# lucidrains/magvit2-pytorch

Hardware: NVIDIA H100
Metric: video-frames/sec tokenize+decode, 17x128x128 bf16 (higher is better)
Workload: dtype bf16

## Files before the change

include/magvit2_b200.h:

```cpp
#ifndef MAGVIT2_B200_H
#define MAGVIT2_B200_H

#include <stddef.h>
#include <stdint.h>

#ifdef __cplusplus
extern "C" {
#endif

#define MV2_ABI_VERSION 4

enum { MV2_F32 = 0, MV2_BF16 = 1,
       MV2_U8 = 2    };
enum { MV2_ACT_NONE = 0, MV2_ACT_ELU = 1, MV2_ACT_SILU = 2,
       MV2_ACT_LEAKY_RELU = 3,
       MV2_ACT_RELU = 4          };
enum { MV2_SHUFFLE_NONE = 0, MV2_SHUFFLE_SPACE = 1, MV2_SHUFFLE_TIME = 2 };
enum {
  MV2_OK = 0,
  MV2_E_ARG = -1,
  MV2_E_CUDA = -2,
  MV2_E_UNSUPPORTED = -3
};

// ... 106 lines not shown
  const void* w;
  const float* bias;
  const void* res;
  void* y;
  int32_t B, Ti, Hi, Wi, Ci;
  int32_t To, Ho, Wo, Co;
  int32_t kt, kh, kw;
  int32_t st, sh, sw;
  int32_t pt, ph, pw;
  int32_t act;
  int32_t shuffle;
  int32_t epi_mode;
  const float* oscale;
  int32_t out_layout;
} mv2_tc_conv_args;
int mv2_tc_conv_supported(const mv2_tc_conv_args* a);
int mv2_tc_conv_forward(const mv2_tc_conv_args* a, void* stream);
int mv2_tc_slab_supported(const mv2_tc_conv_args* a);
int mv2_tc_slab_forward(const mv2_tc_conv_args* a, void* stream);
int mv2_tc_down_space_supported(const mv2_tc_conv_args* a);
int mv2_tc_down_space_forward(const mv2_tc_conv_args* a, void* stream);
int mv2_tc_slab_plan(const mv2_tc_conv_args* a, int n_sm, int* out6);
int mv2_tc_slab_tile(const mv2_tc_conv_args* a, int n_sm, int cta, int k, int* out6);


int mv2_dense_small(const float* x, const float* w, const float* bias, float* y, int B, int K, int N, int act, void* stream);
int mv2_mod_prepare(const float* cond, const float* S, float eps, float* scale_in, float* inv_norm, int B, int Ci, int Co,
                    void* stream);
int mv2_scale_channels(const void* x, const float* scale, void* out, int dtype, int B, int64_t positions_per_clip, int C,
                       void* stream);

typedef struct mv2_tc_ru_args {
  const void* x;
  const void* w3; const float* b3;
  const void* w1; const float* b1;
  const float* se_wk; float se_bk;
  void* y;
  float* se_ws;
  int32_t B, T, H, W, C;
  int32_t kt, kh, kw;
} mv2_tc_ru_args;
int mv2_tc_ru_supported(const mv2_tc_ru_args* a);
int mv2_tc_ru_records(const mv2_tc_ru_args* a);
size_t mv2_tc_ru_workspace_bytes(const mv2_tc_ru_args* a);
int mv2_tc_ru_forward(const mv2_tc_ru_args* a, void* stream);
int mv2_se_gate_records(const void* workspace, int nrec, int F, int C, int Hd,
// ... 25 lines not shown
```

magvit2_pytorch_b200/_lib.py:

```python
from __future__ import annotations

import ctypes as C
import os

_HERE = os.path.dirname(os.path.abspath(__file__))
LIB_PATH = os.environ.get("MV2_LIB_PATH") or os.path.join(_HERE, "libmagvit2_b200.so")

MV2_F32, MV2_BF16, MV2_U8 = 0, 1, 2
ACT_NONE, ACT_ELU, ACT_SILU, ACT_LEAKY_RELU, ACT_RELU = 0, 1, 2, 3, 4
SHUFFLE_NONE, SHUFFLE_SPACE, SHUFFLE_TIME = 0, 1, 2


class Mv2Error(RuntimeError):
    pass


class ConvArgs(C.Structure):
    _fields_ = [
        ("x", C.c_void_p), ("w", C.c_void_p), ("bias", C.c_void_p), ("res", C.c_void_p), ("y", C.c_void_p),
        ("dtype", C.c_int32),
        ("B", C.c_int32), ("Ti", C.c_int32), ("Hi", C.c_int32), ("Wi", C.c_int32), ("Ci", C.c_int32),
        ("To", C.c_int32), ("Ho", C.c_int32), ("Wo", C.c_int32), ("Co", C.c_int32),
        ("kt", C.c_int32), ("kh", C.c_int32), ("kw", C.c_int32),
        ("st", C.c_int32), ("sh", C.c_int32), ("sw", C.c_int32),
# ... 68 lines not shown
    "mv2_geglu": (_I, [_VP, _VP, _I, _I64, _I, _VP]),
    "mv2_lfq_forward": (_I, [_VP, _I, _I64, _I, _I, _I, _VP, _VP, _VP, _VP, _F, _I, _VP, _VP, _VP, _VP]),
    "mv2_lfq_decode": (_I, [_VP, _I, _I64, _I, _I, _I, _VP, _VP, _VP, _I, _VP]),
    "mv2_fsq_forward": (_I, [_VP, _I, _I64, _I, _I, _I, C.POINTER(C.c_int32), _VP, _VP, _VP, _VP, _VP, _VP, _VP, _VP]),
    "mv2_fsq_decode": (_I, [_VP, _I, _I64, _I, _I, _I, C.POINTER(C.c_int32), _VP, _VP, _VP, _I, _VP]),
    "mv2_lfq_entropy_partials": (_I, [_VP, _I64, _I, _I, _F, _VP, _VP, _VP]),
    "mv2_lfq_aux_finalize": (_I, [_VP, _VP, _I, _I, _I64, _I64, _F, _F, _F, _VP, _VP]),
    "mv2_lfq_entropy_fact_workspace_bytes": (_SZ, [_I64, _I, _I]),
    "mv2_lfq_entropy_fact_partials": (_I, [_VP, _I64, _I, _I, _F, _VP, _VP, _VP, _VP]),
    "mv2_lfq_entropy_fact_backward": (_I, [_VP, _VP, _I64, _I, _I, _F, _F, _F, _VP, _VP, _VP]),
    "mv2_gateloop_scan": (_I, [_VP, _VP, _VP, _I, _I, _I, _I, _I, _VP]),
    "mv2_mse": (_I, [_VP, _I, _VP, _I, _I64, _VP, _VP, _VP]),
    "mv2_mse_workspace_bytes": (C.c_size_t, []),
    "mv2_maxpool2x2": (_I, [_VP, _VP, _I, _I, _I, _I, _I, _VP]),
    "mv2_maxpool2x2_backward": (_I, [_VP, _VP, _VP, _I, _I, _I, _I, _I, _VP]),
    "mv2_tc_conv_supported": (_I, [C.POINTER(TcConvArgs)]),
    "mv2_tc_conv_forward": (_I, [C.POINTER(TcConvArgs), _VP]),
    "mv2_tc_slab_supported": (_I, [C.POINTER(TcConvArgs)]),
    "mv2_tc_slab_forward": (_I, [C.POINTER(TcConvArgs), _VP]),
    "mv2_tc_down_space_supported": (_I, [C.POINTER(TcConvArgs)]),
    "mv2_tc_down_space_forward": (_I, [C.POINTER(TcConvArgs), _VP]),
    "mv2_tc_slab_plan": (_I, [C.POINTER(TcConvArgs), _I, C.POINTER(C.c_int32)]),
    "mv2_tc_slab_tile": (_I, [C.POINTER(TcConvArgs), _I, _I, _I, C.POINTER(C.c_int32)]),
    "mv2_dense_small": (_I, [_VP, _VP, _VP, _VP, _I, _I, _I, _I, _VP]),
    "mv2_mod_prepare": (_I, [_VP, _VP, _F, _VP, _VP, _I, _I, _I, _VP]),
    "mv2_scale_channels": (_I, [_VP, _VP, _VP, _I, _I, _I64, _I, _VP]),
    "mv2_tc_ru_supported": (_I, [C.POINTER(TcRuArgs)]),
    "mv2_tc_ru_records": (_I, [C.POINTER(TcRuArgs)]),
    "mv2_tc_ru_workspace_bytes": (_SZ, [C.POINTER(TcRuArgs)]),
    "mv2_tc_ru_forward": (_I, [C.POINTER(TcRuArgs), _VP]),
    "mv2_se_gate_records": (_I, [_VP, _I, _I, _I, _I, _VP, _VP, _VP, _VP, _VP, _VP]),
    "mv2_conv_forward_hist": (_I, [C.POINTER(ConvArgs), C.POINTER(ConvHist), _VP]),
    "mv2_tc_conv_forward_hist": (_I, [C.POINTER(TcConvArgs), C.POINTER(ConvHist), _VP]),
    "mv2_tc_slab_forward_hist": (_I, [C.POINTER(TcConvArgs), C.POINTER(ConvHist), _VP]),
    "mv2_tc_ru_forward_hist": (_I, [C.POINTER(TcRuArgs), C.POINTER(ConvHist), _VP]),
    "mv2_rmsnorm_prev": (_I, [_VP, _VP, _I64, _VP, _I, _VP, _I, _I, _I, _I, _VP]),
    "mv2_attention_tail": (_I, [C.POINTER(AttnArgs), _VP, _I64, _I, _VP, _I64, _VP]),
    "mv2_tc_conv_hist_supported": (_I, [C.POINTER(TcConvArgs)]),
    "mv2_gateloop_scan_state": (_I, [_VP, _VP, _VP, _I, _I, _I, _I, _I, _VP, _VP]),
}

_lib = None


def load():
    global _lib
# ... 26 lines not shown
```

magvit2_pytorch_b200/csrc/tc_common.cuh:

```cuda
#pragma once
#include "common.cuh"
#include <cuda.h>
#include <mutex>

namespace mv2 {


__device__ __forceinline__ uint32_t smem_u32(const void* p) { return (uint32_t)__cvta_generic_to_shared(p); }

__device__ __forceinline__ void mbar_init(uint32_t bar, uint32_t count) {
  asm volatile("mbarrier.init.shared::cta.b64 [%0], %1;" ::"r"(bar), "r"(count));
}
__device__ __forceinline__ void mbar_expect_tx(uint32_t bar, uint32_t bytes) {
  asm volatile("mbarrier.arrive.expect_tx.shared::cta.b64 _, [%0], %1;" ::"r"(bar), "r"(bytes) : "memory");
}
__device__ __forceinline__ void mbar_wait(uint32_t bar, uint32_t parity) {
  asm volatile(
      "{\n\t"
      ".reg .pred P1;\n\t"
      "WAIT_LOOP:\n\t"
      "mbarrier.try_wait.parity.shared::cta.b64 P1, [%0], %1, 0x989680;\n\t"
      "@P1 bra DONE;\n\t"
      "bra WAIT_LOOP;\n\t"
      "DONE:\n\t"
// ... 57 lines not shown
  return ((uint64_t)1 << 16) | ((uint64_t)(sbo >> 4) << 32) | (layout << 62);
}
__device__ __forceinline__ uint32_t desc_lo(uint32_t saddr) { return (saddr & 0x3FFFF) >> 4; }

template <int N> __device__ __forceinline__ void stage_acc(const float (&d)[N / 2], float* stg, int t) {
  const int r = 16 * (t >> 5) + ((t & 31) >> 2), c = 2 * (t & 3);
#pragma unroll
  for (int j = 0; j < N / 8; ++j) {
    *reinterpret_cast<float2*>(stg + r * (N + 4) + 8 * j + c) = make_float2(d[4 * j], d[4 * j + 1]);
    *reinterpret_cast<float2*>(stg + (r + 8) * (N + 4) + 8 * j + c) = make_float2(d[4 * j + 2], d[4 * j + 3]);
  }
}
__device__ __forceinline__ void load_row32(const float* src, int ncols, uint32_t (&r)[32]) {
#pragma unroll
  for (int g = 0; g < 8; ++g) {
    if (g * 4 >= ncols) break;
    const float4 v = *reinterpret_cast<const float4*>(src + 4 * g);
    r[4 * g] = __float_as_uint(v.x); r[4 * g + 1] = __float_as_uint(v.y);
    r[4 * g + 2] = __float_as_uint(v.z); r[4 * g + 3] = __float_as_uint(v.w);
  }
}
__device__ __forceinline__ void named_bar_sync(uint32_t id, uint32_t nthreads) {
  asm volatile("bar.sync %0, %1;" ::"r"(id), "r"(nthreads) : "memory");
}
__device__ __forceinline__ void mbar_arrive(uint32_t bar) {
  asm volatile("mbarrier.arrive.shared::cta.b64 _, [%0];" ::"r"(bar) : "memory");
}

__device__ __forceinline__ uint32_t pack_bf16x2(float a, float b) {
  __nv_bfloat162 v = __floats2bfloat162_rn(a, b);
  return *reinterpret_cast<uint32_t*>(&v);
}



struct TcEpi {
  const float* bias;
  const __nv_bfloat16* res;
  __nv_bfloat16* y;
  int act, shuffle, mode;
  int Co;
  int To, Ho, Wo;
  int out_cf;
  const float* oscale;
};

// ... 31 lines not shown
__device__ __forceinline__ float gelu_fast(float g) {
  const float ag = fabsf(g);
  const float t = rcp_approx(fmaf(0.3275911f * 0.70710678118654752440f, ag, 1.f));
  float p = fmaf(0.5f * 1.061405429f, t, 0.5f * -1.453152027f);
  p = fmaf(p, t, 0.5f * 1.421413741f);
  p = fmaf(p, t, 0.5f * -0.284496736f);
  p = fmaf(p, t, 0.5f * 0.254829592f);
  const float e = ex2_approx((g * g) * (-0.5f * 1.4426950408889634f));
  const float q = (p * t) * e;
  return fmaf(-ag, q, fmaxf(g, 0.f));
}

template <int ACT>
__device__ __forceinline__ float act_ct(float x, bool relu = false) {
  if (ACT == MV2_ACT_ELU) {
    const float e = ex2_approx(x * 1.4426950408889634f) - 1.f;
    return x > 0.f ? x : e;
  }
  if (ACT == MV2_ACT_SILU) return x * rcp_approx(1.f + ex2_approx(-1.4426950408889634f * x));
  if (ACT == MV2_ACT_LEAKY_RELU) return x > 0.f ? x : (relu ? 0.f * x : 0.1f * x);
  return x;
}

template <int MODE, int ACT>
__device__ __forceinline__ void epi_chunk32_t(const TcEpi& e, const uint32_t (&r)[32], int ncols, int n, const float* sb,
                                              int b, int to, int ho, int wo, int64_t row_base, bool relu = false) {
  if (MODE == EPI_GEGLU) {
    const int I = e.Co >> 1;
    const int64_t pos = (((int64_t)b * e.To + to) * e.Ho + ho) * e.Wo + wo;
#pragma unroll
    for (int g = 0; g < 2; ++g) {
      if (g * 16 >= ncols || n + g * 16 >= e.Co) break;
      float v[8];
#pragma unroll
      for (int q = 0; q < 8; ++q) {
        const float xv = __uint_as_float(r[g * 16 + q]) + sb[g * 16 + q];
        const float gt = __uint_as_float(r[g * 16 + 8 + q]) + sb[g * 16 + 8 + q];
        v[q] = gelu_fast(gt) * xv;
      }
      store8_bf16(e.y + pos * I + ((n + g * 16) >> 1), v);
    }
    return;
  }
  const int cy = MODE == EPI_SHUFFLE ? (e.shuffle == MV2_SHUFFLE_SPACE ? (e.Co >> 2) : (e.Co >> 1)) : e.Co;
  const bool vec_ok = (cy & 7) == 0;
#pragma unroll
  for (int g = 0; g < 4; ++g) {
    const int ng = n + g * 8;
    if (g * 8 >= ncols || ng >= e.Co) break;
    float v[8];
    {
      const float4 b0 = *reinterpret_cast<const float4*>(sb + g * 8), b1 = *reinterpret_cast<const float4*>(sb + g * 8 + 4);
      const float bb[8] = {b0.x, b0.y, b0.z, b0.w, b1.x, b1.y, b1.z, b1.w};
      if (MODE != EPI_SHUFFLE && e.oscale) {
#pragma unroll
        for (int q = 0; q < 8; ++q) {
          const float os = ng + q < e.Co ? e.oscale[(int64_t)b * e.Co + ng + q] : 0.f;
          v[q] = act_ct<ACT>(__uint_as_float(r[g * 8 + q]) * os + bb[q], relu);
        }
      } else
#pragma unroll
      for (int q = 0; q < 8; ++q) v[q] = act_ct<ACT>(__uint_as_float(r[g * 8 + q]) + bb[q], relu);
// ... 51 lines not shown
__device__ __forceinline__ void epi_act32_t(uint32_t (&r)[32], const float* sb, bool relu = false) {
#pragma unroll
  for (int g = 0; g < 8; ++g) {
    const float4 b = *reinterpret_cast<const float4*>(sb + g * 4);
    r[4 * g] = __float_as_uint(act_ct<ACT>(__uint_as_float(r[4 * g]) + b.x, relu));
    r[4 * g + 1] = __float_as_uint(act_ct<ACT>(__uint_as_float(r[4 * g + 1]) + b.y, relu));
    r[4 * g + 2] = __float_as_uint(act_ct<ACT>(__uint_as_float(r[4 * g + 2]) + b.z, relu));
    r[4 * g + 3] = __float_as_uint(act_ct<ACT>(__uint_as_float(r[4 * g + 3]) + b.w, relu));
  }
}
__device__ __forceinline__ void epi_act32(int act, uint32_t (&r)[32], const float* sb) {
  if (act == MV2_ACT_ELU) epi_act32_t<MV2_ACT_ELU>(r, sb);
  else if (act == MV2_ACT_SILU) epi_act32_t<MV2_ACT_SILU>(r, sb);
  else if (act == MV2_ACT_LEAKY_RELU || act == MV2_ACT_RELU) epi_act32_t<MV2_ACT_LEAKY_RELU>(r, sb, act == MV2_ACT_RELU);
  else epi_act32_t<MV2_ACT_NONE>(r, sb);
}
__device__ __forceinline__ void epi_pack32(int act, const uint32_t (&r)[32], const float* sb, uint32_t (&pk)[16]) {
  if (act == MV2_ACT_ELU) epi_pack32_t<MV2_ACT_ELU>(r, sb, pk);
  else if (act == MV2_ACT_SILU) epi_pack32_t<MV2_ACT_SILU>(r, sb, pk);
  else if (act == MV2_ACT_LEAKY_RELU || act == MV2_ACT_RELU) epi_pack32_t<MV2_ACT_LEAKY_RELU>(r, sb, pk, act == MV2_ACT_RELU);
  else epi_pack32_t<MV2_ACT_NONE>(r, sb, pk);
}

template <int MODE>
__device__ __forceinline__ void epi_chunk32(const TcEpi& e, const uint32_t (&r)[32], int ncols, int n, const float* sb,
                                            int b, int to, int ho, int wo, int64_t row_base) {
  if (MODE == EPI_GEGLU) { epi_chunk32_t<EPI_GEGLU, MV2_ACT_NONE>(e, r, ncols, n, sb, b, to, ho, wo, row_base); return; }
  if (e.act == MV2_ACT_ELU) epi_chunk32_t<MODE, MV2_ACT_ELU>(e, r, ncols, n, sb, b, to, ho, wo, row_base);
  else if (e.act == MV2_ACT_SILU) epi_chunk32_t<MODE, MV2_ACT_SILU>(e, r, ncols, n, sb, b, to, ho, wo, row_base);
  else if (e.act == MV2_ACT_LEAKY_RELU || e.act == MV2_ACT_RELU)
    epi_chunk32_t<MODE, MV2_ACT_LEAKY_RELU>(e, r, ncols, n, sb, b, to, ho, wo, row_base, e.act == MV2_ACT_RELU);
  else epi_chunk32_t<MODE, MV2_ACT_NONE>(e, r, ncols, n, sb, b, to, ho, wo, row_base);
}

typedef CUresult (*EncodeTiledFn)(CUtensorMap*, CUtensorMapDataType, cuuint32_t, void*, const cuuint64_t*,
                                  const cuuint64_t*, const cuuint32_t*, const cuuint32_t*, CUtensorMapInterleave,
                                  CUtensorMapSwizzle, CUtensorMapL2promotion, CUtensorMapFloatOOBfill);

static inline EncodeTiledFn get_encode_fn() {
  static EncodeTiledFn fn = nullptr;
  static std::once_flag once;
  std::call_once(once, [] {
    void* f = nullptr;
    cudaDriverEntryPointQueryResult q;
    if (cudaGetDriverEntryPoint("cuTensorMapEncodeTiled", &f, cudaEnableDefault, &q) == cudaSuccess &&
        q == cudaDriverEntryPointSuccess)
// ... 34 lines not shown
```

magvit2_pytorch_b200/csrc/tc_slab.cu:

```cuda
#include "common.cuh"
#include "tc_common.cuh"
#include <cuda.h>
#include <algorithm>
#include <type_traits>
#include <mutex>
#include <map>
#include <vector>
#include <string.h>

namespace mv2 {

struct alignas(64) SlabParams {
  CUtensorMap amap;
  CUtensorMap hmap;
  CUtensorMap wmap;
  CUtensorMap wmap2;
  int kt, kh, kw, pt, ph, pw;
  int st;
  int hist_T;
  int Ci, kchunks, row_bytes;
  int B, T, H, W, Co;
  int mw, pitch, slab_h, slab_bytes, slab_stride;
  int bn, n_tiles_n, tiles_w, tiles_h, total_tiles;
  int slab_stages, w_stages;
// ... 467 lines not shown
          const int h20 = c.h0 + sub * 4;
          const int64_t row0 = ((((int64_t)c.b * p.T + c.t) * p.H + h20) * p.W + w2) * p.Co + c.n0 + piece * 8;
          const int64_t kstride = (int64_t)p.W * p.Co;
          const int kmax = w2 < p.W ? p.H - h20 : 0;
          for (int c0 = ((j + half) & 1) * 32; c0 < p.bn; c0 += 64) {
            uint32_t r[32], pk[16];
            uint4 rv[4];
            if (MODE == EPI_PLAIN_RES) {
              const __nv_bfloat16* rr = p.epi.res + row_base + c.n0 + c0;
#pragma unroll
              for (int g = 0; g < 4; ++g)
                rv[g] = (row_ok && c.n0 + c0 + g * 8 < p.Co && c0 + g * 8 < p.bn) ? *reinterpret_cast<const uint4*>(rr + g * 8) : make_uint4(0, 0, 0, 0);
            }
            load_row32(srow + c0, 32, r);
            if ((MODE == EPI_PLAIN || MODE == EPI_PLAIN_RES) && p.epi.oscale) {
              const float* os = p.epi.oscale + (int64_t)c.b * p.Co + c.n0 + c0;
#pragma unroll
              for (int i = 0; i < 32; ++i) r[i] = __float_as_uint(__uint_as_float(r[i]) * (c.n0 + c0 + i < p.Co ? os[i] : 0.f));
            }
            if (MODE == EPI_PLAIN_RES) {
              epi_act32(p.epi.act, r, sbias + c.n0 + c0);
              const float rs = p.epi.mode == 2 ? 0.70710678118654752440f : 1.f;
#pragma unroll
              for (int g = 0; g < 4; ++g) {
                const uint32_t w4[4] = {rv[g].x, rv[g].y, rv[g].z, rv[g].w};
#pragma unroll
                for (int q = 0; q < 4; ++q)
                  pk[4 * g + q] = pack_bf16x2((__uint_as_float(r[8 * g + 2 * q]) + __uint_as_float(w4[q] << 16)) * rs,
                                              (__uint_as_float(r[8 * g + 2 * q + 1]) + __uint_as_float(w4[q] & 0xffff0000u)) * rs);
              }
            } else
            epi_pack32(p.epi.act, r, sbias + c.n0 + c0, pk);
#pragma unroll
            for (int g = 0; g < 4; ++g)
              asm volatile("st.shared.v4.b32 [%0], {%1, %2, %3, %4};" ::"r"(wr + ((g ^ wsw) << 4)), "r"(pk[4 * g]),
                           "r"(pk[4 * g + 1]), "r"(pk[4 * g + 2]), "r"(pk[4 * g + 3]) : "memory");
            __syncwarp();
            const bool col_ok = c.n0 + c0 + piece * 8 < p.Co && c0 + piece * 8 < p.bn;
            const int klim = col_ok ? kmax : 0;
            __nv_bfloat16* yp;
            int64_t ks;
            if (MODE == EPI_SHUFFLE_ST) {
              const int n = c.n0 + c0;
              if (p.epi.shuffle == MV2_SHUFFLE_SPACE) {
                const int cy = p.Co >> 2, qd = n / cy, cb = n - qd * cy;
                yp = p.epi.y + ((((int64_t)c.b * p.T + c.t) * (2 * p.H) + (2 * h20 + (qd >> 1))) * (2 * p.W) + (2 * w2 + (qd & 1))) * cy + cb + piece * 8;
                ks = (int64_t)4 * p.W * cy;
              } else {
                const int cy = p.Co >> 1, qd = n / cy, cb = n - qd * cy;
                yp = p.epi.y + ((((int64_t)c.b * (2 * p.T) + (2 * c.t + qd)) * p.H + h20) * p.W + w2) * cy + cb + piece * 8;
                ks = (int64_t)p.W * cy;
              }
            } else {
              yp = p.epi.y + row0 + c0;
              ks = kstride;
            }
#pragma unroll
            for (int k = 0; k < 4; ++k) {
              uint4 v;
              asm volatile("ld.shared.v4.b32 {%0, %1, %2, %3}, [%4];" : "=r"(v.x), "=r"(v.y), "=r"(v.z), "=r"(v.w)
                           : "r"(rd + k * 512 + ((piece ^ (((8 * k + rl) >> 1) & 3)) << 4)));
              if (k < klim) *reinterpret_cast<uint4*>(yp + k * ks) = v;
            }
            __syncwarp();
          }
        } else {
          for (int c0 = ((j + half) & 1) * 32; c0 < p.bn; c0 += 64) {
            uint32_t r[32];
            load_row32(srow + c0, 32, r);
            if (row_ok) epi_chunk32<MODE>(p.epi, r, min(32, p.bn - c0), c.n0 + c0, sbias + c.n0 + c0, c.b, c.t, h, w, row_base);
          }
        }
      }
    }
  }
}

}

using namespace mv2;

extern "C" int mv2_tc_slab_supported(const mv2_tc_conv_args* a) {
  if (!a) return 0;
  if (a->sh != 1 || a->sw != 1) return 0;
// ... 304 lines not shown
```

magvit2_pytorch_b200/engine.py:

```python
from __future__ import annotations

import ctypes as C
from dataclasses import dataclass
from typing import Dict, List, Optional, Tuple

import torch

from . import _lib
from ._lib import (ACT_ELU, ACT_NONE, ACT_SILU, MV2_BF16, MV2_F32, MV2_U8, SHUFFLE_NONE, SHUFFLE_SPACE,
                   SHUFFLE_TIME, AttnArgs, ConvArgs, ConvHist, TcConvArgs, TcRuArgs, check)


def _dt(t: torch.dtype) -> int:
    if t == torch.float32:
        return MV2_F32
    if t == torch.bfloat16:
        return MV2_BF16
    raise TypeError(f"unsupported dtype {t} (only float32 and bfloat16)")


def _src_dt(t: torch.dtype) -> int:
    return MV2_U8 if t == torch.uint8 else _dt(t)


def _ptr(t: Optional[torch.Tensor]):
    return None if t is None else t.data_ptr()


class AttnDropout:

    def __init__(self, p: float, seed: int):
        self.p, self.seed, self.calls = float(p), int(seed), 0

# ... 134 lines not shown
    return pk


def param_signature(module):
    ps = list(module.parameters())
    return (tuple((p.data_ptr(), p._version) for p in ps), ps[0].dtype, ps[0].device)


class Engine:

    def __init__(self, model):
        self.model = model
        self.lib = _lib.load()
        self._packs: Dict[str, object] = {}
        self._sig = None
        self._sig_id = 0
        self.launches = 0
        self.use_tc = True
        self.tc_variant = "auto"
        self.fuse_ru = True
        self.fused_ru_calls = 0
        self.tc_calls = 0
        self.slab_calls = 0
        self.simt_conv_calls = 0
        self.taps: Optional[dict] = None
        self._prof: Optional[list] = None
        self.conv_log: Optional[list] = None
        self.dropout: Optional[AttnDropout] = None

    def bind(self, p0: torch.Tensor, what: str):
        if p0.device.type != "cuda":
            raise RuntimeError(f"{what} runs on CUDA (sm_90a) only; move the model with .cuda() -- there is no CPU fallback")
        if p0.dtype not in (torch.float32, torch.bfloat16):
            raise TypeError("parameters must be float32 or bfloat16")
        arch = self.lib.mv2_device_arch()
        if arch != 90:
            raise RuntimeError(f"libmagvit2_b200.so targets sm_90a (H100); device reports sm_{arch}")
        self.dtype = p0.dtype
        self.device = p0.device

    def prepare(self):
        sig = param_signature(self.model)
        if sig == self._sig:
            return
        m = self.model
        self.bind(m.conv_in.conv.weight, "magvit2_pytorch_b200.VideoTokenizer")
# ... 100 lines not shown
            hist = ConvHist(h=t.data_ptr() + t0 * fe * t.element_size(), T_h=n, clip_stride=t.shape[1] * fe)

        def advance():
            T = x.shape[1]
            if T >= need or h is None:
                keep = min(need, T)
                ss.put("hist", (x, T - keep, keep))
                return
            t, t0, n = h
            old = min(n, need - T)
            buf = self._new((x.shape[0], old + T) + tuple(x.shape[2:]), x.dtype)
            self.copy_frames(t, t0 + n - old, old, dst=buf, dst_t0=0)
            self.copy_frames(x, 0, T, dst=buf, dst_t0=old)
            ss.put("hist", (buf, 0, old + T))
        return hist, advance

    def _hist_cat(self, ss: StreamState, x):
        t, t0, n = ss.get("hist")
        cat = self._new((x.shape[0], n + x.shape[1]) + tuple(x.shape[2:]), x.dtype)
        self.copy_frames(t, t0, n, dst=cat, dst_t0=0)
        self.copy_frames(x, 0, x.shape[1], dst=cat, dst_t0=n)
        return cat

    def conv(self, x, pk: ConvPack, *, stride=(1, 1, 1), pad=None, out_spatial=None, act=ACT_NONE,
             res=None, shuffle=SHUFFLE_NONE, token_shift=False, out_cf=False, oscale=None, ss: Optional[StreamState] = None):
        B, Ti, Hi, Wi, Ci = x.shape
        hist, advance = self._conv_hist(ss, x, pk.k[0] - 1)
        tc_ok = (self.dtype == torch.bfloat16 and self.use_tc and pk.w_tc is not None and not token_shift
                 and Ci == pk.Ci_tc)
        kt, kh, kw = pk.k_tc if (tc_ok and pk.k_tc) else pk.k
        if pad is None:
            pad = (kt - 1, kh // 2, kw // 2)
        if out_spatial is None:
            out_spatial = (Ti, Hi, Wi)
        To, Ho, Wo = out_spatial
        if tc_ok:
            co_gemm = pk.Co_tc
            co_out = co_gemm // 2 if pk.epi_mode == 1 else co_gemm
            if shuffle == SHUFFLE_SPACE:
                y = self._new((B, To, 2 * Ho, 2 * Wo, co_out // 4))
            elif shuffle == SHUFFLE_TIME:
                y = self._new((B, 2 * To, Ho, Wo, co_out // 2))
            elif out_cf:
                y = self._new((B, co_out, To, Ho, Wo))
            else:
                y = self._new((B, To, Ho, Wo, co_out))
            if res is not None:
                assert res.shape == y.shape and res.dtype == y.dtype and res.is_contiguous()
            ta = TcConvArgs(x=_ptr(x), w=_ptr(pk.w_tc), bias=_ptr(pk.bias_tc), res=_ptr(res), y=_ptr(y),
                            B=B, Ti=Ti, Hi=Hi, Wi=Wi, Ci=Ci, To=To, Ho=Ho, Wo=Wo, Co=co_gemm,
                            kt=kt, kh=kh, kw=kw, st=stride[0], sh=stride[1], sw=stride[2],
                            pt=pad[0], ph=pad[1], pw=pad[2], act=act, shuffle=shuffle, epi_mode=pk.epi_mode,
                            oscale=_ptr(oscale), out_layout=int(out_cf))
            use_slab = self.tc_variant != "tap" and bool(self.lib.mv2_tc_slab_supported(C.byref(ta)))
            use_down = (not use_slab and self.tc_variant != "tap" and pk.w_down is not None and stride == (1, 2, 2)
                        and bool(self.lib.mv2_tc_down_space_supported(C.byref(ta))))
            if use_down:
                ta.w = _ptr(pk.w_down)
                use_slab = True
            if use_slab or self.lib.mv2_tc_conv_supported(C.byref(ta)):
                if self._prof is not None:
                    e0, e1 = torch.cuda.Event(enable_timing=True), torch.cuda.Event(enable_timing=True)
                    e0.record()
                if use_down:
                    check(self.lib.mv2_tc_down_space_forward(C.byref(ta), self._stream()), "mv2_tc_down_space_forward")
                    self.slab_calls += 1
                elif use_slab and hist is not None:
                    check(self.lib.mv2_tc_slab_forward_hist(C.byref(ta), C.byref(hist), self._stream()), "mv2_tc_slab_forward_hist")
                    self.slab_calls += 1
                elif use_slab:
                    check(self.lib.mv2_tc_slab_forward(C.byref(ta), self._stream()), "mv2_tc_slab_forward")
                    self.slab_calls += 1
                elif hist is not None and self.lib.mv2_tc_conv_hist_supported(C.byref(ta)):
                    check(self.lib.mv2_tc_conv_forward_hist(C.byref(ta), C.byref(hist), self._stream()), "mv2_tc_conv_forward_hist")
                elif hist is not None:
                    cat = self._hist_cat(ss, x)
                    ta.x, ta.Ti, ta.pt = _ptr(cat), cat.shape[1], pad[0] - hist.T_h
                    check(self.lib.mv2_tc_conv_forward(C.byref(ta), self._stream()), "mv2_tc_conv_forward")
                else:
                    check(self.lib.mv2_tc_conv_forward(C.byref(ta), self._stream()), "mv2_tc_conv_forward")
                if self._prof is not None:
                    e1.record()
                    self._prof.append((e0, e1, 2.0 * B * To * Ho * Wo * pk.macs,
                                       "slab" if use_slab else "tap", pk.k[1] * pk.k[2] * pk.k[0]))
                if self.conv_log is not None:
                    self.conv_log.append(dict(kind="slab" if use_slab else "tap", Ci=Ci, Co=co_out, k=tuple(pk.k), out=(B, To, Ho, Wo),
                                              geglu=pk.epi_mode == 1, shuffle=shuffle, res=res is not None, act=act,
                                              epi_mode=pk.epi_mode, stride=tuple(stride)))
                self.launches += 1
                self.tc_calls += 1
                if advance is not None:
                    advance()
                return y
            assert not out_cf, "channels-first output is a wgmma slab-kernel feature"
            assert pk.w is not None and pk.epi_mode in (0, 2) and Ci == pk.Ci, "wgmma-only weight pack has no CUDA-core fallback"
            kt, kh, kw = pk.k
        assert Ci == pk.Ci, (Ci, pk.Ci)
        assert pk.w is not None and not out_cf
        if shuffle == SHUFFLE_SPACE:
            y = self._new((B, To, 2 * Ho, 2 * Wo, pk.Co // 4))
        elif shuffle == SHUFFLE_TIME:
            y = self._new((B, 2 * To, Ho, Wo, pk.Co // 2))
        else:
            y = self._new((B, To, Ho, Wo, pk.Co))
        if res is not None:
            assert res.shape == y.shape and res.dtype == y.dtype and res.is_contiguous()
        self.simt_conv_calls += 1
        a = ConvArgs(x=_ptr(x), w=_ptr(pk.w), bias=_ptr(pk.bias), res=_ptr(res), y=_ptr(y), dtype=_dt(self.dtype),
                     B=B, Ti=Ti, Hi=Hi, Wi=Wi, Ci=Ci, To=To, Ho=Ho, Wo=Wo, Co=pk.Co,
# ... 491 lines not shown
```

Baseline: 4961.

## Add persistent warp-specialized TMA/wgmma GEMM kernel for pointwise 1x1x1 convs

Adds a dedicated persistent GEMM kernel for 1x1x1 stride-1 convolutions. It uses a TMA producer warp, a multi-stage mbarrier ring and two consumer warpgroups that alternate tiles via named barriers, with fused GEGLU, residual and pixel-shuffle epilogues. The engine routes eligible slab convs to it when the tile count fills at least one wave of SMs. The aim is to replace the general slab conv path for pointwise layers with a simpler, better pipelined GEMM. In exchange it adds a new kernel with its own epilogue code paths, and the epilogue helpers shared with the slab kernel are refactored into common functions.

```diff
diff --git a/include/magvit2_b200.h b/include/magvit2_b200.h
--- a/include/magvit2_b200.h
+++ b/include/magvit2_b200.h
@@ -152,6 +152,10 @@
 int mv2_tc_down_space_forward(const mv2_tc_conv_args* a, void* stream);
 int mv2_tc_slab_plan(const mv2_tc_conv_args* a, int n_sm, int* out6);
 int mv2_tc_slab_tile(const mv2_tc_conv_args* a, int n_sm, int cta, int k, int* out6);
+int mv2_tc_gemm_supported(const mv2_tc_conv_args* a);
+int mv2_tc_gemm_forward(const mv2_tc_conv_args* a, void* stream);
+int mv2_tc_gemm_plan(const mv2_tc_conv_args* a, int n_sm, int* out6);
+int mv2_tc_gemm_tile(const mv2_tc_conv_args* a, int n_sm, int cta, int k, int* out4);
 
 
 int mv2_dense_small(const float* x, const float* w, const float* bias, float* y, int B, int K, int N, int act, void* stream);
diff --git a/magvit2_pytorch_b200/_lib.py b/magvit2_pytorch_b200/_lib.py
--- a/magvit2_pytorch_b200/_lib.py
+++ b/magvit2_pytorch_b200/_lib.py
@@ -114,6 +114,10 @@
     "mv2_tc_down_space_forward": (_I, [C.POINTER(TcConvArgs), _VP]),
     "mv2_tc_slab_plan": (_I, [C.POINTER(TcConvArgs), _I, C.POINTER(C.c_int32)]),
     "mv2_tc_slab_tile": (_I, [C.POINTER(TcConvArgs), _I, _I, _I, C.POINTER(C.c_int32)]),
+    "mv2_tc_gemm_supported": (_I, [C.POINTER(TcConvArgs)]),
+    "mv2_tc_gemm_forward": (_I, [C.POINTER(TcConvArgs), _VP]),
+    "mv2_tc_gemm_plan": (_I, [C.POINTER(TcConvArgs), _I, C.POINTER(C.c_int32)]),
+    "mv2_tc_gemm_tile": (_I, [C.POINTER(TcConvArgs), _I, _I, _I, C.POINTER(C.c_int32)]),
     "mv2_dense_small": (_I, [_VP, _VP, _VP, _VP, _I, _I, _I, _I, _VP]),
     "mv2_mod_prepare": (_I, [_VP, _VP, _F, _VP, _VP, _I, _I, _I, _VP]),
     "mv2_scale_channels": (_I, [_VP, _VP, _VP, _I, _I, _I64, _I, _VP]),
diff --git a/magvit2_pytorch_b200/csrc/tc_common.cuh b/magvit2_pytorch_b200/csrc/tc_common.cuh
--- a/magvit2_pytorch_b200/csrc/tc_common.cuh
+++ b/magvit2_pytorch_b200/csrc/tc_common.cuh
@@ -103,6 +103,9 @@
 }
 __device__ __forceinline__ void named_bar_sync(uint32_t id, uint32_t nthreads) {
   asm volatile("bar.sync %0, %1;" ::"r"(id), "r"(nthreads) : "memory");
+}
+__device__ __forceinline__ void named_bar_arrive(uint32_t id, uint32_t nthreads) {
+  asm volatile("bar.arrive %0, %1;" ::"r"(id), "r"(nthreads) : "memory");
 }
 __device__ __forceinline__ void mbar_arrive(uint32_t bar) {
   asm volatile("mbarrier.arrive.shared::cta.b64 _, [%0];" ::"r"(bar) : "memory");
@@ -180,6 +183,15 @@
   return x;
 }
 
+__device__ __forceinline__ void geglu8(const uint32_t (&r)[32], int g, const float* sb, float (&v)[8]) {
+#pragma unroll
+  for (int q = 0; q < 8; ++q) {
+    const float xv = __uint_as_float(r[g * 16 + q]) + sb[g * 16 + q];
+    const float gt = __uint_as_float(r[g * 16 + 8 + q]) + sb[g * 16 + 8 + q];
+    v[q] = gelu_fast(gt) * xv;
+  }
+}
+
 template <int MODE, int ACT>
 __device__ __forceinline__ void epi_chunk32_t(const TcEpi& e, const uint32_t (&r)[32], int ncols, int n, const float* sb,
                                               int b, int to, int ho, int wo, int64_t row_base, bool relu = false) {
@@ -190,12 +202,7 @@
     for (int g = 0; g < 2; ++g) {
       if (g * 16 >= ncols || n + g * 16 >= e.Co) break;
       float v[8];
-#pragma unroll
-      for (int q = 0; q < 8; ++q) {
-        const float xv = __uint_as_float(r[g * 16 + q]) + sb[g * 16 + q];
-        const float gt = __uint_as_float(r[g * 16 + 8 + q]) + sb[g * 16 + 8 + q];
-        v[q] = gelu_fast(gt) * xv;
-      }
+      geglu8(r, g, sb, v);
       store8_bf16(e.y + pos * I + ((n + g * 16) >> 1), v);
     }
     return;
@@ -293,6 +300,27 @@
   else epi_pack32_t<MV2_ACT_NONE>(r, sb, pk);
 }
 
+__device__ __forceinline__ void epi_res_pack8(const uint32_t (&r)[32], int g, uint4 rv, float rs, uint32_t (&pk)[16]) {
+  const uint32_t w4[4] = {rv.x, rv.y, rv.z, rv.w};
+#pragma unroll
+  for (int q = 0; q < 4; ++q)
+    pk[4 * g + q] = pack_bf16x2((__uint_as_float(r[8 * g + 2 * q]) + __uint_as_float(w4[q] << 16)) * rs,
+                                (__uint_as_float(r[8 * g + 2 * q + 1]) + __uint_as_float(w4[q] & 0xffff0000u)) * rs);
+}
+
+__device__ __forceinline__ void xpose_put64(uint32_t wr, uint32_t wsw, const uint32_t (&pk)[16]) {
+#pragma unroll
+  for (int g = 0; g < 4; ++g)
+    asm volatile("st.shared.v4.b32 [%0], {%1, %2, %3, %4};" ::"r"(wr + ((g ^ wsw) << 4)), "r"(pk[4 * g]),
+                 "r"(pk[4 * g + 1]), "r"(pk[4 * g + 2]), "r"(pk[4 * g + 3]) : "memory");
+}
+__device__ __forceinline__ uint4 xpose_get16(uint32_t rd, int k, int rl, int piece) {
+  uint4 v;
+  asm volatile("ld.shared.v4.b32 {%0, %1, %2, %3}, [%4];" : "=r"(v.x), "=r"(v.y), "=r"(v.z), "=r"(v.w)
+               : "r"(rd + k * 512 + ((piece ^ (((8 * k + rl) >> 1) & 3)) << 4)));
+  return v;
+}
+
 template <int MODE>
 __device__ __forceinline__ void epi_chunk32(const TcEpi& e, const uint32_t (&r)[32], int ncols, int n, const float* sb,
                                             int b, int to, int ho, int wo, int64_t row_base) {
diff --git a/magvit2_pytorch_b200/csrc/tc_gemm.cu b/magvit2_pytorch_b200/csrc/tc_gemm.cu
--- /dev/null
+++ b/magvit2_pytorch_b200/csrc/tc_gemm.cu
@@ -0,0 +1,318 @@
+#include "common.cuh"
+#include "tc_common.cuh"
+#include <cuda.h>
+#include <algorithm>
+#include <string.h>
+
+namespace mv2 {
+
+constexpr int GEMM_BM = 128, GEMM_BN = 128, GEMM_BK = 64;
+constexpr uint32_t GEMM_A_BYTES = GEMM_BM * GEMM_BK * 2, GEMM_STAGE_BYTES = GEMM_A_BYTES + GEMM_BN * GEMM_BK * 2;
+constexpr int GEMM_STG_PITCH = 32 + 4;
+constexpr int GEMM_MAX_STAGES = 8;
+constexpr int GEMM_PRODUCER_REGS = 40, GEMM_CONSUMER_REGS = 232;
+
+struct alignas(64) GemmParams {
+  CUtensorMap amap;
+  CUtensorMap wmap;
+  int M, Ci, Co, kchunks;
+  int n_tiles_n, m_tiles, total_tiles, stages;
+  int T, H, W;
+  TcEpi epi;
+};
+
+__host__ __device__ __forceinline__ int gemm_tile_of_cta(const GemmParams& p, int k, int cta, int grid) {
+  const int64_t tile = (int64_t)k * grid + cta;
+  return tile < p.total_tiles ? (int)tile : -1;
+}
+
+struct GemmSmem { uint32_t bar, sbias, stg, end; };
+__host__ __device__ __forceinline__ GemmSmem gemm_smem_layout(const GemmParams& p, uint32_t base) {
+  GemmSmem m;
+  m.bar = base + (uint32_t)p.stages * GEMM_STAGE_BYTES;
+  m.sbias = (m.bar + 16u * p.stages + 15u) & ~15u;
+  m.stg = m.sbias + (uint32_t)p.n_tiles_n * GEMM_BN * 4;
+  m.end = m.stg + 2u * GEMM_BM * GEMM_STG_PITCH * 4;
+  return m;
+}
+
+template <int MODE>
+__global__ void __launch_bounds__(384, 1) tc_gemm_kernel(const __grid_constant__ GemmParams p) {
+  extern __shared__ uint8_t smem_raw[];
+  const uint32_t ring = (smem_u32(smem_raw) + 1023u) & ~1023u;
+  const GemmSmem L = gemm_smem_layout(p, ring);
+  auto gen = [&](uint32_t u) { return smem_raw + (u - smem_u32(smem_raw)); };
+  const int warp = threadIdx.x >> 5, lane = threadIdx.x & 31;
+  const uint32_t full = L.bar, empty = L.bar + 8 * p.stages;
+  const uint32_t stages = (uint32_t)p.stages;
+  float* sbias = reinterpret_cast<float*>(gen(L.sbias));
+
+  if (threadIdx.x == 0) {
+    for (int s = 0; s < p.stages; ++s) { mbar_init(full + 8 * s, 1); mbar_init(empty + 8 * s, 4); }
+    fence_barrier_init();
+  }
+  if (warp == 0 && lane == 0) { tma_prefetch_desc(&p.amap); tma_prefetch_desc(&p.wmap); }
+  if (warp >= 4) {
+    const int nb = p.n_tiles_n * GEMM_BN;
+    for (int i = threadIdx.x - 128; i < nb; i += 256) sbias[i] = (p.epi.bias && i < p.Co) ? p.epi.bias[i] : 0.f;
+  }
+  __syncthreads();
+  pdl_wait();
+  pdl_launch_dependents();
+
+  if (warp < 4) {
+    setmaxnreg_dec<GEMM_PRODUCER_REGS>();
+    if (warp == 0 && lane == 0) {
+      uint32_t s = 0, ph = 0;
+      for (int k = 0, tile; (tile = gemm_tile_of_cta(p, k, blockIdx.x, gridDim.x)) >= 0; ++k) {
+        const int m0 = tile / p.n_tiles_n * GEMM_BM, n0 = tile % p.n_tiles_n * GEMM_BN;
+        for (int kc = 0; kc < p.kchunks; ++kc) {
+          mbar_wait(empty + 8 * s, ph ^ 1);
+          mbar_expect_tx(full + 8 * s, GEMM_STAGE_BYTES);
+          const uint32_t st = ring + s * GEMM_STAGE_BYTES;
+          tma_load_2d(st, &p.amap, full + 8 * s, kc * GEMM_BK, m0);
+          tma_load_2d(st + GEMM_A_BYTES, &p.wmap, full + 8 * s, kc * GEMM_BK, n0);
+          if (++s == stages) { s = 0; ph ^= 1; }
+        }
+      }
+    }
+  } else {
+    setmaxnreg_inc<GEMM_CONSUMER_REGS>();
+    const int wg = (warp - 4) >> 2, wq = warp & 3, tid = threadIdx.x & 127;
+    const uint32_t wg_bar = 1 + wg, my_turn = 3 + wg, other_turn = 4 - wg;
+    float* stg = reinterpret_cast<float*>(gen(L.stg)) + wg * GEMM_BM * GEMM_STG_PITCH;
+    const uint32_t xbuf = smem_u32(stg) + (uint32_t)wq * 32 * GEMM_STG_PITCH * 4;
+    const int rl = lane >> 2, piece = lane & 3;
+    const uint32_t wr = xbuf + lane * 64, wsw = (lane >> 1) & 3, rd = xbuf + rl * 64;
+    const uint64_t d_hi = gmma_desc_hi(8 * 128, 128);
+    const int cy = p.epi.shuffle == MV2_SHUFFLE_SPACE ? (p.Co >> 2) : (p.Co >> 1);
+    float acc[2][GEMM_BN / 2];
+
+    for (int k = wg, tile; (tile = gemm_tile_of_cta(p, k, blockIdx.x, gridDim.x)) >= 0; k += 2) {
+      const int m0 = tile / p.n_tiles_n * GEMM_BM, n0 = tile % p.n_tiles_n * GEMM_BN;
+      const uint32_t pos = (uint32_t)k * (uint32_t)p.kchunks;
+      uint32_t s = pos % stages, par = (pos / stages) & 1u, prev = 0, accum = 0;
+      if (MODE == EPI_PLAIN_RES && m0 + tid < p.M) {
+        const __nv_bfloat16* rr = p.epi.res + (int64_t)(m0 + tid) * p.Co + n0;
+        asm volatile("prefetch.global.L2 [%0];" ::"l"(rr) : "memory");
+        if (n0 + 64 < p.Co) asm volatile("prefetch.global.L2 [%0];" ::"l"(rr + 64) : "memory");
+      }
+      if (k > 0) named_bar_sync(my_turn, 256);
+      for (int kc = 0; kc < p.kchunks; ++kc) {
+        mbar_wait(full + 8 * s, par);
+        wgmma_fence();
+        const uint32_t lo = desc_lo(ring + s * GEMM_STAGE_BYTES);
+        const uint64_t bd = d_hi | (uint64_t)(lo + (GEMM_A_BYTES >> 4));
+#pragma unroll
+        for (int j = 0; j < 2; ++j) {
+          const uint64_t ad = d_hi | (uint64_t)(lo + j * ((64 * 128) >> 4));
+          wgmma_bf16<GEMM_BN>(acc[j], ad, bd, accum);
+          wgmma_bf16<GEMM_BN>(acc[j], ad + 2, bd + 2, 1u);
+          wgmma_bf16<GEMM_BN>(acc[j], ad + 4, bd + 4, 1u);
+          wgmma_bf16<GEMM_BN>(acc[j], ad + 6, bd + 6, 1u);
+        }
+        wgmma_commit();
+        wgmma_wait<1>();
+        if (kc > 0) {
+          __syncwarp();
+          if (lane == 0) mbar_arrive(empty + 8 * prev);
+        }
+        prev = s;
+        accum = 1;
+        if (++s == stages) { s = 0; par ^= 1; }
+      }
+      if (gemm_tile_of_cta(p, k + 1, blockIdx.x, gridDim.x) >= 0) named_bar_arrive(other_turn, 256);
+      wgmma_wait<0>();
+      __syncwarp();
+      if (lane == 0) mbar_arrive(empty + 8 * prev);
+
+      const int mrow = m0 + tid;
+      const int mst = m0 + 32 * wq + rl;
+      int spos[MODE == EPI_SHUFFLE_ST ? 4 : 1];
+      uint32_t gpk[16];
+#pragma unroll
+      for (int c = 0; c < GEMM_BN / 32; ++c) {
+        const int c0 = 32 * c, n = n0 + c0;
+        if (n >= p.Co && (MODE != EPI_GEGLU || (c & 1) == 0)) break;
+        named_bar_sync(wg_bar, 128);
+        {
+          const int r = 16 * (tid >> 5) + ((tid & 31) >> 2), cc = 2 * (tid & 3);
+#pragma unroll
+          for (int j = 0; j < 2; ++j)
+#pragma unroll
+            for (int i = 0; i < 4; ++i) {
+              const int jj = 4 * c + i;
+              *reinterpret_cast<float2*>(stg + (64 * j + r) * GEMM_STG_PITCH + 8 * i + cc) = make_float2(acc[j][4 * jj], acc[j][4 * jj + 1]);
+              *reinterpret_cast<float2*>(stg + (64 * j + r + 8) * GEMM_STG_PITCH + 8 * i + cc) = make_float2(acc[j][4 * jj + 2], acc[j][4 * jj + 3]);
+            }
+        }
+        named_bar_sync(wg_bar, 128);
+        if (MODE == EPI_SHUFFLE_ST && c == 0)
+#pragma unroll
+          for (int q = 0; q < 4; ++q) {
+            const int m = mst + 8 * q;
+            const int w = m % p.W, r1 = m / p.W, h = r1 % p.H, bt = r1 / p.H;
+            if (p.epi.shuffle == MV2_SHUFFLE_SPACE) spos[q] = (bt * (2 * p.H) + 2 * h) * (2 * p.W) + 2 * w;
+            else spos[q] = (((bt / p.T) * (2 * p.T) + 2 * (bt % p.T)) * p.H + h) * p.W + w;
+          }
+        uint32_t r[32];
+        if (MODE == EPI_GEGLU) {
+          load_row32(stg + tid * GEMM_STG_PITCH, 32, r);
+#pragma unroll
+          for (int g = 0; g < 2; ++g) {
+            float v[8];
+            geglu8(r, g, sbias + n, v);
+#pragma unroll
+            for (int i = 0; i < 4; ++i) gpk[8 * (c & 1) + 4 * g + i] = pack_bf16x2(v[2 * i], v[2 * i + 1]);
+          }
+          if ((c & 1) == 0) continue;
+          __syncwarp();
+          xpose_put64(wr, wsw, gpk);
+          __syncwarp();
+          const int I = p.Co >> 1, np = n - 32;
+          const bool col_ok = np + 16 * piece < p.Co;
+#pragma unroll
+          for (int q = 0; q < 4; ++q) {
+            const uint4 v = xpose_get16(rd, q, rl, piece);
+            if (col_ok && mst + 8 * q < p.M)
+              *reinterpret_cast<uint4*>(p.epi.y + (int64_t)(mst + 8 * q) * I + (np >> 1) + piece * 8) = v;
+          }
+          continue;
+        }
+        load_row32(stg + tid * GEMM_STG_PITCH, 32, r);
+        uint32_t pk[16];
+        if (MODE == EPI_PLAIN_RES) {
+          epi_act32(p.epi.act, r, sbias + n);
+          const float rs = p.epi.mode == 2 ? 0.70710678118654752440f : 1.f;
+          const __nv_bfloat16* rr = p.epi.res + (int64_t)mrow * p.Co + n;
+#pragma unroll
+          for (int g = 0; g < 4; ++g) {
+            const uint4 rv = (mrow < p.M && n + g * 8 < p.Co) ? *reinterpret_cast<const uint4*>(rr + g * 8) : make_uint4(0, 0, 0, 0);
+            epi_res_pack8(r, g, rv, rs, pk);
+          }
+        } else {
+          epi_pack32(p.epi.act, r, sbias + n, pk);
+        }
+        __syncwarp();
+        xpose_put64(wr, wsw, pk);
+        __syncwarp();
+        int64_t coff = n + piece * 8;
+        if (MODE == EPI_SHUFFLE_ST) {
+          const int qd = n / cy, cb = n - qd * cy;
+          coff = (p.epi.shuffle == MV2_SHUFFLE_SPACE ? ((int64_t)(qd >> 1) * (2 * p.W) + (qd & 1)) * cy
+                                                      : (int64_t)qd * p.H * p.W * cy) + cb + piece * 8;
+        }
+        const bool col_ok = n + piece * 8 < p.Co;
+#pragma unroll
+        for (int q = 0; q < 4; ++q) {
+          const uint4 v = xpose_get16(rd, q, rl, piece);
+          const int64_t off = (MODE == EPI_SHUFFLE_ST ? (int64_t)spos[q & (MODE == EPI_SHUFFLE_ST ? 3 : 0)] * cy
+                                                      : (int64_t)(mst + 8 * q) * p.Co) + coff;
+          if (col_ok && mst + 8 * q < p.M) *reinterpret_cast<uint4*>(p.epi.y + off) = v;
+        }
+      }
+    }
+  }
+}
+
+}
+
+using namespace mv2;
+
+extern "C" int mv2_tc_gemm_supported(const mv2_tc_conv_args* a) {
+  if (!a) return 0;
+  if (a->kt != 1 || a->kh != 1 || a->kw != 1 || a->st != 1 || a->sh != 1 || a->sw != 1) return 0;
+  if (a->pt != 0 || a->ph != 0 || a->pw != 0) return 0;
+  if (a->To != a->Ti || a->Ho != a->Hi || a->Wo != a->Wi || a->out_layout != 0 || a->oscale) return 0;
+  if (a->B < 1 || a->To < 1 || a->Ho < 1 || a->Wo < 1) return 0;
+  if ((int64_t)a->B * a->To * a->Ho * a->Wo >= ((int64_t)1 << 31)) return 0;
+  if (a->Ci % 64 != 0 || a->Ci < 64 || a->Co % 8 != 0 || a->Co < 8 || a->Co > 4096) return 0;
+  if (a->epi_mode < 0 || a->epi_mode > 2) return 0;
+  if (a->epi_mode == 1 && (a->Co % 16 != 0 || a->res || a->shuffle != MV2_SHUFFLE_NONE)) return 0;
+  if (a->epi_mode == 2 && (!a->res || a->shuffle != MV2_SHUFFLE_NONE)) return 0;
+  if (a->shuffle != MV2_SHUFFLE_NONE) {
+    if (a->shuffle != MV2_SHUFFLE_SPACE && a->shuffle != MV2_SHUFFLE_TIME) return 0;
+    if (a->res || (a->shuffle == MV2_SHUFFLE_SPACE ? a->Co / 4 : a->Co / 2) % 32 != 0) return 0;
+    if ((int64_t)a->B * a->To * a->Ho * a->Wo * 4 >= ((int64_t)1 << 31)) return 0;
+  }
+  return 1;
+}
+
+static int gemm_fill_plan(const mv2_tc_conv_args* a, GemmParams& p) {
+  memset(&p, 0, sizeof(p));
+  p.M = a->B * a->To * a->Ho * a->Wo;
+  p.Ci = a->Ci; p.Co = a->Co; p.kchunks = a->Ci / GEMM_BK;
+  p.T = a->To; p.H = a->Ho; p.W = a->Wo;
+  p.n_tiles_n = ceil_div(a->Co, GEMM_BN);
+  p.m_tiles = ceil_div(p.M, GEMM_BM);
+  MV2_CHECK_ARG((int64_t)p.n_tiles_n * p.m_tiles < ((int64_t)1 << 31));
+  p.total_tiles = p.n_tiles_n * p.m_tiles;
+  p.epi = tc_epi_of(a);
+  p.stages = 1;
+  const uint32_t rest = gemm_smem_layout(p, 0).end - GEMM_STAGE_BYTES;
+  p.stages = std::min<int>(GEMM_MAX_STAGES, (int)((227 * 1024 - 1024 - rest - 16 * GEMM_MAX_STAGES) / GEMM_STAGE_BYTES));
+  MV2_CHECK_ARG(p.stages >= 4);
+  return MV2_OK;
+}
+
+static size_t gemm_smem_bytes(const GemmParams& p) { return 1024 + gemm_smem_layout(p, 0).end; }
+
+extern "C" int mv2_tc_gemm_plan(const mv2_tc_conv_args* a, int n_sm, int* out6) {
+  MV2_CHECK_ARG(a && out6 && n_sm > 0);
+  if (!mv2_tc_gemm_supported(a)) { set_error("mv2_tc_gemm_plan: unsupported shape"); return MV2_E_UNSUPPORTED; }
+  GemmParams p;
+  if (const int rc = gemm_fill_plan(a, p)) return rc;
+  out6[0] = p.m_tiles; out6[1] = p.n_tiles_n; out6[2] = p.total_tiles; out6[3] = std::min(p.total_tiles, n_sm);
+  out6[4] = p.stages; out6[5] = p.kchunks;
+  return MV2_OK;
+}
+
+extern "C" int mv2_tc_gemm_tile(const mv2_tc_conv_args* a, int n_sm, int cta, int k, int* out4) {
+  MV2_CHECK_ARG(a && out4 && n_sm > 0 && cta >= 0 && k >= 0);
+  if (!mv2_tc_gemm_supported(a)) { set_error("mv2_tc_gemm_tile: unsupported shape"); return MV2_E_UNSUPPORTED; }
+  GemmParams p;
+  if (const int rc = gemm_fill_plan(a, p)) return rc;
+  const int grid = std::min(p.total_tiles, n_sm);
+  MV2_CHECK_ARG(cta < grid);
+  const int tile = gemm_tile_of_cta(p, k, cta, grid);
+  out4[0] = tile;
+  out4[1] = tile >= 0 ? tile / p.n_tiles_n * GEMM_BM : -1;
+  out4[2] = tile >= 0 ? tile % p.n_tiles_n * GEMM_BN : -1;
+  out4[3] = tile >= 0 ? (k & 1) : -1;
+  return MV2_OK;
+}
+
+extern "C" int mv2_tc_gemm_forward(const mv2_tc_conv_args* a, void* stream) {
+  MV2_CHECK_ARG(a && a->x && a->w && a->y);
+  if (!mv2_tc_gemm_supported(a)) { set_error("mv2_tc_gemm_forward: unsupported shape"); return MV2_E_UNSUPPORTED; }
+  GemmParams p;
+  if (const int rc = gemm_fill_plan(a, p)) return rc;
+  const cuuint64_t xdims[2] = {(cuuint64_t)a->Ci, (cuuint64_t)p.M}, wdims[2] = {(cuuint64_t)a->Ci, (cuuint64_t)a->Co};
+  const cuuint64_t strides[1] = {(cuuint64_t)a->Ci * 2};
+  const cuuint32_t box[2] = {GEMM_BK, GEMM_BM};
+  if (const int rc = encode_bf16_map(&p.amap, 2, a->x, xdims, strides, box, CU_TENSOR_MAP_SWIZZLE_128B, "gemm x")) return rc;
+  if (const int rc = encode_bf16_map(&p.wmap, 2, a->w, wdims, strides, box, CU_TENSOR_MAP_SWIZZLE_128B, "gemm w")) return rc;
+  int mode = EPI_PLAIN;
+  if (a->epi_mode == 1) mode = EPI_GEGLU;
+  else if (a->shuffle != MV2_SHUFFLE_NONE) mode = EPI_SHUFFLE_ST;
+  else if (a->res) mode = EPI_PLAIN_RES;
+  static void (*const kernels[])(GemmParams) = {tc_gemm_kernel<EPI_PLAIN>, tc_gemm_kernel<EPI_GEGLU>,
+                                                tc_gemm_kernel<EPI_PLAIN_RES>, tc_gemm_kernel<EPI_SHUFFLE_ST>};
+  const int ki = mode == EPI_PLAIN ? 0 : mode == EPI_GEGLU ? 1 : mode == EPI_PLAIN_RES ? 2 : 3;
+  static PerDeviceOnce attr_once;
+  const cudaError_t attr_err = attr_once.run([] {
+    cudaError_t e = cudaSuccess;
+    for (auto k : kernels)
+      if (e == cudaSuccess) e = cudaFuncSetAttribute(k, cudaFuncAttributeMaxDynamicSharedMemorySize, 227 * 1024);
+    return e;
+  });
+  if (attr_err != cudaSuccess) { set_error("cudaFuncSetAttribute failed: %s", cudaGetErrorString(attr_err)); return MV2_E_CUDA; }
+  const size_t smem = gemm_smem_bytes(p);
+  MV2_CHECK_ARG(smem <= 227 * 1024);
+  int dev = 0, n_sm = 132;
+  cudaGetDevice(&dev);
+  cudaDeviceGetAttribute(&n_sm, cudaDevAttrMultiProcessorCount, dev);
+  launch_k(kernels[ki], dim3(std::min(p.total_tiles, n_sm)), dim3(384), smem, (cudaStream_t)stream, p);
+  MV2_CHECK_LAUNCH();
+  return MV2_OK;
+}
diff --git a/magvit2_pytorch_b200/csrc/tc_slab.cu b/magvit2_pytorch_b200/csrc/tc_slab.cu
--- a/magvit2_pytorch_b200/csrc/tc_slab.cu
+++ b/magvit2_pytorch_b200/csrc/tc_slab.cu
@@ -513,19 +513,10 @@
               epi_act32(p.epi.act, r, sbias + c.n0 + c0);
               const float rs = p.epi.mode == 2 ? 0.70710678118654752440f : 1.f;
 #pragma unroll
-              for (int g = 0; g < 4; ++g) {
-                const uint32_t w4[4] = {rv[g].x, rv[g].y, rv[g].z, rv[g].w};
-#pragma unroll
-                for (int q = 0; q < 4; ++q)
-                  pk[4 * g + q] = pack_bf16x2((__uint_as_float(r[8 * g + 2 * q]) + __uint_as_float(w4[q] << 16)) * rs,
-                                              (__uint_as_float(r[8 * g + 2 * q + 1]) + __uint_as_float(w4[q] & 0xffff0000u)) * rs);
-              }
+              for (int g = 0; g < 4; ++g) epi_res_pack8(r, g, rv[g], rs, pk);
             } else
-            epi_pack32(p.epi.act, r, sbias + c.n0 + c0, pk);
-#pragma unroll
-            for (int g = 0; g < 4; ++g)
-              asm volatile("st.shared.v4.b32 [%0], {%1, %2, %3, %4};" ::"r"(wr + ((g ^ wsw) << 4)), "r"(pk[4 * g]),
-                           "r"(pk[4 * g + 1]), "r"(pk[4 * g + 2]), "r"(pk[4 * g + 3]) : "memory");
+              epi_pack32(p.epi.act, r, sbias + c.n0 + c0, pk);
+            xpose_put64(wr, wsw, pk);
             __syncwarp();
             const bool col_ok = c.n0 + c0 + piece * 8 < p.Co && c0 + piece * 8 < p.bn;
             const int klim = col_ok ? kmax : 0;
@@ -548,9 +539,7 @@
             }
 #pragma unroll
             for (int k = 0; k < 4; ++k) {
-              uint4 v;
-              asm volatile("ld.shared.v4.b32 {%0, %1, %2, %3}, [%4];" : "=r"(v.x), "=r"(v.y), "=r"(v.z), "=r"(v.w)
-                           : "r"(rd + k * 512 + ((piece ^ (((8 * k + rl) >> 1) & 3)) << 4)));
+              const uint4 v = xpose_get16(rd, k, rl, piece);
               if (k < klim) *reinterpret_cast<uint4*>(yp + k * ks) = v;
             }
             __syncwarp();
diff --git a/magvit2_pytorch_b200/engine.py b/magvit2_pytorch_b200/engine.py
--- a/magvit2_pytorch_b200/engine.py
+++ b/magvit2_pytorch_b200/engine.py
@@ -9,6 +9,8 @@
 from . import _lib
 from ._lib import (ACT_ELU, ACT_NONE, ACT_SILU, MV2_BF16, MV2_F32, MV2_U8, SHUFFLE_NONE, SHUFFLE_SPACE,
                    SHUFFLE_TIME, AttnArgs, ConvArgs, ConvHist, TcConvArgs, TcRuArgs, check)
+
+GEMM_MIN_WAVES = 1
 
 
 def _dt(t: torch.dtype) -> int:
@@ -189,6 +191,7 @@
         self.fused_ru_calls = 0
         self.tc_calls = 0
         self.slab_calls = 0
+        self.gemm_calls = 0
         self.simt_conv_calls = 0
         self.taps: Optional[dict] = None
         self._prof: Optional[list] = None
@@ -335,6 +338,14 @@
         self.copy_frames(x, 0, x.shape[1], dst=cat, dst_t0=n)
         return cat
 
+    def _gemm_routes(self, ta) -> bool:
+        if not self.lib.mv2_tc_gemm_supported(C.byref(ta)):
+            return False
+        n_sm = torch.cuda.get_device_properties(torch.cuda.current_device()).multi_processor_count
+        plan = (C.c_int32 * 6)()
+        check(self.lib.mv2_tc_gemm_plan(C.byref(ta), n_sm, plan), "mv2_tc_gemm_plan")
+        return plan[2] >= GEMM_MIN_WAVES * n_sm
+
     def conv(self, x, pk: ConvPack, *, stride=(1, 1, 1), pad=None, out_spatial=None, act=ACT_NONE,
              res=None, shuffle=SHUFFLE_NONE, token_shift=False, out_cf=False, oscale=None, ss: Optional[StreamState] = None):
         B, Ti, Hi, Wi, Ci = x.shape
@@ -366,6 +377,7 @@
                             pt=pad[0], ph=pad[1], pw=pad[2], act=act, shuffle=shuffle, epi_mode=pk.epi_mode,
                             oscale=_ptr(oscale), out_layout=int(out_cf))
             use_slab = self.tc_variant != "tap" and bool(self.lib.mv2_tc_slab_supported(C.byref(ta)))
+            use_gemm = use_slab and self._gemm_routes(ta)
             use_down = (not use_slab and self.tc_variant != "tap" and pk.w_down is not None and stride == (1, 2, 2)
                         and bool(self.lib.mv2_tc_down_space_supported(C.byref(ta))))
             if use_down:
@@ -375,7 +387,10 @@
                 if self._prof is not None:
                     e0, e1 = torch.cuda.Event(enable_timing=True), torch.cuda.Event(enable_timing=True)
                     e0.record()
-                if use_down:
+                if use_gemm:
+                    check(self.lib.mv2_tc_gemm_forward(C.byref(ta), self._stream()), "mv2_tc_gemm_forward")
+                    self.gemm_calls += 1
+                elif use_down:
                     check(self.lib.mv2_tc_down_space_forward(C.byref(ta), self._stream()), "mv2_tc_down_space_forward")
                     self.slab_calls += 1
                 elif use_slab and hist is not None:
@@ -392,12 +407,12 @@
                     check(self.lib.mv2_tc_conv_forward(C.byref(ta), self._stream()), "mv2_tc_conv_forward")
                 else:
                     check(self.lib.mv2_tc_conv_forward(C.byref(ta), self._stream()), "mv2_tc_conv_forward")
+                kind = "gemm" if use_gemm else ("slab" if use_slab else "tap")
                 if self._prof is not None:
                     e1.record()
-                    self._prof.append((e0, e1, 2.0 * B * To * Ho * Wo * pk.macs,
-                                       "slab" if use_slab else "tap", pk.k[1] * pk.k[2] * pk.k[0]))
+                    self._prof.append((e0, e1, 2.0 * B * To * Ho * Wo * pk.macs, kind, pk.k[1] * pk.k[2] * pk.k[0]))
                 if self.conv_log is not None:
-                    self.conv_log.append(dict(kind="slab" if use_slab else "tap", Ci=Ci, Co=co_out, k=tuple(pk.k), out=(B, To, Ho, Wo),
+                    self.conv_log.append(dict(kind=kind, Ci=Ci, Co=co_out, k=tuple(pk.k), out=(B, To, Ho, Wo),
                                               geglu=pk.epi_mode == 1, shuffle=shuffle, res=res is not None, act=act,
                                               epi_mode=pk.epi_mode, stride=tuple(stride)))
                 self.launches += 1
```

New measurement: 5207, median of 6. 1.05x the previous value.
